# zju3dv/pats

Hardware: AMD Instinct MI355X
Metric: image-pairs/sec (coarse+fine OT) on 640x480 MegaDepth; OT iters/sec per pair (higher is better)
Workload: dtype f32 (contractions: fp32 operands split into fp16 hi + lo, three exact-product MFMA passes, fp32 accumulate)

## Files before the change

### include/pats_amd.h

```cpp
#ifndef PATS_AMD_H
#define PATS_AMD_H

#include <stddef.h>
#include <stdint.h>

#ifdef __cplusplus
extern "C" {
#endif

typedef void* pats_stream_t;

enum {
    PATS_OK = 0,
    PATS_ERR_INVALID = 1,
    PATS_ERR_UNSUPPORTED = 2,
    PATS_ERR_LAUNCH = 3,
    PATS_ERR_NO_DEVICE = 4
};

enum { PATS_SINKHORN_AUTO = 0, PATS_SINKHORN_LOG = 1, PATS_SINKHORN_KERNEL = 2 };

const char* pats_version(void);
#define PATS_ABI_VERSION 8
int pats_abi_version(void);
// ... 230 lines not shown
int pats_third_inputs_f32(const uint8_t* if_nomatching, const float* pts, int64_t B, float* mkpts0,
                          float* mkpts1, int64_t* b_ids, int64_t capacity, int64_t* count, void* workspace,
                          size_t workspace_bytes, pats_stream_t stream);

int pats_refine_scatter_f32(const uint8_t* if_nomatching, const float* pts, const float* mkpts1_f,
                            const float* label, int label_stride, int64_t B, int64_t P,
                            uint8_t* if_nomatching16, float* pts16, void* workspace,
                            size_t workspace_bytes, pats_stream_t stream);

size_t pats_get_result_workspace_bytes(int64_t cells0, int64_t rows1, int64_t cells1);
int pats_get_result_f32(int batch_size, const uint8_t* if_nomatching0, const uint8_t* if_nomatching1,
                        int64_t rows1, const float* average_point0, const float* average_point1,
                        const float* scale0, const float* scale1, int64_t scale1_cell_stride,
                        const int* patch_size0, const int* patch_size1, const uint8_t* left_choice0,
                        const uint8_t* left_choice1, float* matches_l, float* matches_r, int64_t capacity,
                        int64_t* count, void* workspace, size_t workspace_bytes, pats_stream_t stream);

int pats_get_result_chunks_f32(int Cmax, int64_t pairs, const uint8_t* masks, const uint8_t* if_nomatching16,
                               int64_t rows_cap, const float* pts_new, const float* pts16, const float* scales,
                               const int* patch_size0, const int* patch_size1, const uint8_t* left_choice0,
                               const uint8_t* left_choice1, float* matches_l, float* matches_r, int32_t* match_row,
                               int64_t capacity, int64_t* count, void* workspace, size_t workspace_bytes,
                               pats_stream_t stream);

size_t pats_matches_by_pair_workspace_bytes(int Cmax, int64_t pairs);
int pats_matches_by_pair_f32(const float* matches_l, const float* matches_r, const int32_t* match_row, const int64_t* M_dev,
                             const int32_t* row_cell, const int64_t* chunk_base, int Cmax, int64_t pairs, int N,
                             float* out_l, float* out_r, int64_t* pair_off, void* workspace, size_t workspace_bytes,
                             pats_stream_t stream);
int pats_matches_by_pair_summary_f32(const float* matches_l, const float* matches_r, const int32_t* match_row, const int64_t* M_dev,
                                     const int32_t* row_cell, const int64_t* chunk_base, int Cmax, int64_t pairs, int N,
                                     float* out_l, float* out_r, int64_t* pair_off, const int64_t* P_dev, const int32_t* status,
                                     void* workspace, size_t workspace_bytes, pats_stream_t stream);

typedef struct pats_pair_table {
    int64_t pairs;
    const int32_t* shape_host;
    const int64_t* cell_base_host;
    const int32_t* shape;
    const int64_t* cell_base;
    const int64_t* img_base;
} pats_pair_table_t;

int pats_chunk_rows_ragged(const pats_pair_table_t* tab, const uint8_t* if_nomatching1, int if_local, int Cmax, int64_t rows_cap,
                           int32_t* sum_cycle, int32_t* cycle_num, int64_t* second, int64_t* third, uint8_t* masks,
                           int64_t* chunk_base, int64_t* crop_base, int32_t* row_cell, int32_t* row_pair, uint8_t* row_forced,
                           int32_t* row_crop, int32_t* row_slot, int32_t* status, void* workspace, size_t workspace_bytes,
                           pats_stream_t stream);
int pats_compute_imgs_bounds_ragged_f32(const pats_pair_table_t* tab, const float* x_scale, const float* y_scale,
                                        const float* average_point, const uint8_t* if_nomatching, int64_t* bound5, int64_t* K_img,
                                        int64_t* K_total, float* x_scale_new, float* y_scale_new, float* average_new,
                                        pats_stream_t stream);
int pats_left_crops_ragged_f32(const pats_pair_table_t* tab, const float* left, const int64_t* bound5, int64_t K_cap,
                               const int64_t* K_dev, float* out, pats_stream_t stream);
int pats_tensor_resize_hwc_ragged_f32(const pats_pair_table_t* tab, const float* right, int margin, const int64_t* bound5,
                                      int64_t K_cap, const int64_t* K_dev, float* out, int32_t* status, pats_stream_t stream);

typedef enum { PATS_IMG_F32 = 0, PATS_IMG_F16 = 1, PATS_IMG_BF16 = 2, PATS_IMG_U8 = 3 } pats_img_dtype_t;
typedef enum { PATS_CROP_HWC = 0, PATS_CROP_CHW = 1 } pats_crop_layout_t;
typedef struct pats_crop_format {
    int32_t dtype;
    int32_t layout;
    int32_t normalize;
    float mean[3];
    float std[3];
} pats_crop_format_t;
// ... 309 lines not shown
```

### pats_amd/_lib.py

```python
import ctypes
import os

_HERE = os.path.dirname(os.path.abspath(__file__))
LIB_PATH = os.path.join(_HERE, "libpats_amd.so")
if os.environ.get("PATS_AMD_DIAG_LIB", "") not in ("", "0"):
    _sfx = os.environ["PATS_AMD_DIAG_LIB"]
    LIB_PATH = os.path.join(_HERE, "libpats_amd_diag%s.so" % ("" if _sfx == "1" else _sfx))

c_void_p, c_int, c_i64, c_f, c_size = (ctypes.c_void_p, ctypes.c_int, ctypes.c_int64, ctypes.c_float,
                                       ctypes.c_size_t)

ABI_VERSION = 8



class PairTable(ctypes.Structure):
    _fields_ = [("pairs", ctypes.c_int64), ("shape_host", c_void_p), ("cell_base_host", c_void_p), ("shape", c_void_p),
                ("cell_base", c_void_p), ("img_base", c_void_p)]


_TAB = ctypes.POINTER(PairTable)


class CropFormat(ctypes.Structure):
# ... 124 lines not shown
                                          c_i64, c_void_p, c_int, c_int, c_void_p, c_void_p, c_void_p] + [c_void_p] * 10 +
                                  [c_void_p, c_size, c_void_p]),
    "pats_get_result_chunks_f32": (c_int, [c_int, c_i64, c_void_p, c_void_p, c_i64, c_void_p, c_void_p, c_void_p,
                                           ctypes.POINTER(c_int), ctypes.POINTER(c_int), c_void_p, c_void_p, c_void_p,
                                           c_void_p, c_void_p, c_i64, c_void_p, c_void_p, c_size, c_void_p]),
    "pats_merge_workspace_bytes": (c_size, [c_i64, c_int, c_int, c_int]),
    "pats_merge_patches": (c_int, [c_int, c_i64, c_void_p, c_int, c_int, c_int, c_void_p, c_void_p, c_void_p,
                                   c_void_p, c_void_p, c_size, c_void_p]),
    "pats_compact_workspace_bytes": (c_size, [c_i64]),
    "pats_third_inputs_f32": (c_int, [c_void_p, c_void_p, c_i64, c_void_p, c_void_p, c_void_p, c_i64, c_void_p,
                                      c_void_p, c_size, c_void_p]),
    "pats_refine_scatter_f32": (c_int, [c_void_p, c_void_p, c_void_p, c_void_p, c_int, c_i64, c_i64, c_void_p,
                                        c_void_p, c_void_p, c_size, c_void_p]),
    "pats_attention_f32": (c_int, [c_void_p, c_void_p, c_void_p, c_i64, c_int, c_int, c_int, c_int, c_void_p, c_void_p,
                                   c_void_p]),
    "pats_attentional_propagation_workspace_bytes": (c_size, [c_i64, c_int, c_int, c_int]),
    "pats_attentional_propagation_f32": (c_int, [c_void_p, c_void_p, c_i64, c_int, c_int, c_int, c_int, c_void_p, c_int, c_f,
                                                 c_void_p, c_void_p, c_void_p, c_size, c_void_p]),
    "pats_propagation_packed_bytes": (c_size, [c_int, c_int]),
    "pats_propagation_pack_f32": (c_int, [c_void_p, c_int, c_int, c_void_p, c_size, c_void_p]),
    "pats_attentional_propagation_packed_f32": (c_int, [c_void_p, c_void_p, c_i64, c_int, c_int, c_int, c_int, c_void_p, c_void_p,
                                                        c_int, c_f, c_void_p, c_void_p, c_void_p, c_size, c_void_p]),
    "pats_attentional_gnn_packed_workspace_bytes": (c_size, [c_i64, c_int, c_int, c_int]),
    "pats_attentional_gnn_packed_f32": (c_int, [c_void_p, c_void_p, c_i64, c_void_p, c_i64, c_int, c_int, c_int, c_int, c_void_p, c_void_p,
                                                c_void_p, c_f, c_void_p, c_void_p, c_void_p, c_size, c_void_p]),
    "pats_attentional_propagation_packed_counted_f32": (c_int, [c_void_p, c_void_p, c_i64, c_void_p, c_i64, c_int, c_int, c_int, c_int,
                                                                c_void_p, c_void_p, c_int, c_f, c_void_p, c_void_p, c_void_p, c_size,
                                                                c_void_p]),
    "pats_matches_by_pair_workspace_bytes": (c_size, [c_int, c_i64]),
    "pats_matches_by_pair_f32": (c_int, [c_void_p, c_void_p, c_void_p, c_void_p, c_void_p, c_void_p, c_int, c_i64, c_int,
                                         c_void_p, c_void_p, c_void_p, c_void_p, c_size, c_void_p]),
    "pats_matches_by_pair_summary_f32": (c_int, [c_void_p, c_void_p, c_void_p, c_void_p, c_void_p, c_void_p, c_int, c_i64, c_int,
                                                 c_void_p, c_void_p, c_void_p, c_void_p, c_void_p, c_void_p, c_size, c_void_p]),
    "pats_chunk_rows_ragged": (c_int, [_TAB, c_void_p, c_int, c_int, c_i64] + [c_void_p] * 14 + [c_size, c_void_p]),
    "pats_compute_imgs_bounds_ragged_f32": (c_int, [_TAB] + [c_void_p] * 10 + [c_void_p]),
    "pats_left_crops_ragged_f32": (c_int, [_TAB, c_void_p, c_void_p, c_i64, c_void_p, c_void_p, c_void_p]),
    "pats_tensor_resize_hwc_ragged_f32": (c_int, [_TAB, c_void_p, c_int, c_void_p, c_i64, c_void_p, c_void_p, c_void_p, c_void_p]),
    "pats_left_crops_typed": (c_int, [_TAB, c_void_p, c_int, c_int, c_int, c_int, c_int, c_int, c_void_p, c_i64, c_void_p,
                                      _FMT, c_void_p, c_void_p]),
    "pats_tensor_resize_hwc_typed": (c_int, [_TAB, c_void_p, c_int, c_int, c_int, c_int, c_int, c_void_p, c_i64, c_void_p, _FMT,
                                             c_void_p, c_void_p, c_void_p]),
    "pats_tensor_resize_typed": (c_int, [c_void_p, c_int, c_int, c_int, c_int, c_int, c_void_p, c_i64, c_void_p, _FMT, c_void_p,
                                         c_void_p, c_void_p]),
    "pats_merge_ragged_workspace_bytes": (c_size, [c_i64]),
    "pats_merge_patches_ragged": (c_int, [_TAB, c_int, c_int, c_i64] + [c_void_p] * 8 + [c_int, c_void_p, c_void_p, c_size, c_void_p]),
    "pats_get_result_chunks_ragged_f32": (c_int, [_TAB, c_int, c_void_p, c_void_p, c_i64, c_void_p, c_void_p, c_void_p,
                                                  ctypes.POINTER(c_int), c_void_p, c_void_p, c_void_p, c_void_p, c_void_p, c_i64,
                                                  c_void_p, c_void_p, c_size, c_void_p]),
    "pats_matches_by_row_pair_summary_f32": (c_int, [c_void_p, c_void_p, c_void_p, c_void_p, c_void_p, c_void_p, c_int, c_i64,
                                                     c_void_p, c_void_p, c_void_p, c_void_p, c_void_p, c_void_p, c_size, c_void_p]),
    "pats_prepare_images_max_side": (c_i64, []),
    "pats_prepare_images_u8": (c_int, [c_void_p, c_void_p, c_i64, c_void_p, c_i64, c_void_p, c_i64, c_int, c_void_p]),
    "pats_third_level_typed_conf": (c_int, [c_void_p, c_void_p, c_int, c_i64, c_void_p, c_int, c_void_p, c_void_p, c_void_p, c_void_p,
                                            c_void_p, c_int, c_int, c_void_p, c_void_p, c_void_p, c_void_p, c_void_p, c_void_p,
                                            c_void_p]),
    "pats_compute_result_ws_conf_f32": (c_int, [c_void_p, c_int, c_i64, c_void_p, c_void_p, c_void_p, c_void_p,
                                                c_int, c_void_p, c_void_p, c_void_p, c_void_p, c_void_p, c_void_p,
                                                c_void_p, c_size, c_void_p]),
    "pats_refine_scatter_conf_f32": (c_int, [c_void_p, c_void_p, c_void_p, c_void_p, c_int, c_void_p, c_i64, c_i64, c_void_p,
                                             c_void_p, c_void_p, c_void_p, c_size, c_void_p]),
    "pats_get_result_chunks_conf_f32": (c_int, [c_int, c_i64, c_void_p, c_void_p, c_i64, c_void_p, c_void_p, c_void_p, c_void_p,
                                                ctypes.POINTER(c_int), ctypes.POINTER(c_int), c_void_p, c_void_p, c_void_p,
                                                c_void_p, c_void_p, c_void_p, c_i64, c_void_p, c_void_p, c_size, c_void_p]),
    "pats_get_result_chunks_ragged_conf_f32": (c_int, [_TAB, c_int, c_void_p, c_void_p, c_i64, c_void_p, c_void_p, c_void_p, c_void_p,
                                                       ctypes.POINTER(c_int), c_void_p, c_void_p, c_void_p, c_void_p, c_void_p,
                                                       c_void_p, c_i64, c_void_p, c_void_p, c_size, c_void_p]),
# ... 128 lines not shown
```

### pats_amd/batch.py

```python
import numpy as np
import torch

from . import ops


class Capacities:

    def __init__(self, pairs, h, w, if_local=True, p_cap_per_pair=None, rows_cap=None):
        self.pairs, self.h, self.w = int(pairs), int(h), int(w)
        self.N = self.h * self.w
        self.chunk_cap = 2 * self.w if if_local else 512
        self.Cmax = ops.max_chunks(self.h, self.w, self.chunk_cap)
        self.rows_cap = self.pairs * (self.N + (self.Cmax - 1) * self.w) if rows_cap is None else int(rows_cap)
        per_pair = int(1.25 * 16 * self.N) if p_cap_per_pair is None else int(p_cap_per_pair)
        self.P_cap = self.pairs * per_pair


class MixedCapacities:

    def __init__(self, shapes, if_local=True, p_cap_per_pair=None, rows_cap=None):
        self.shapes = [(int(h), int(w)) for h, w in shapes]
        self.if_local = bool(if_local)
        if not self.shapes:
            raise ValueError("MixedCapacities: no pairs")
# ... 163 lines not shown
    if events is not None:
        em = torch.cuda.Event(enable_timing=True)
        em.record()
        events.setdefault("fine_mid", []).append(em)
        ops.set_cost_ot_mid_event(em)
    live = rows.chunk_base[-1:]
    Z2, cflag2 = ops.cost_ot(f0, f1, 2, _one(f0.device), ns2, iters, bias_k=2.0 if if_outdoor else 3.0, return_flags=True,
                             count=live)
    if e is not None:
        e.record()
    trust2, pts2, _, _, ifn_L2, _ = ops.est_position_second(Z2, sx, sy, [96, 96], 8, col_nomatch=cflag2, count=live)
    merged = ops.merge_patches_batch(merge_new, rows, trust2, (H, W), ifn_L2)
    mk0, mk1, b_ids, P = ops.third_inputs(merged, pts2, capacity=cap.P_cap, sync=False)
    return {"co": co, "merged": merged, "pts2": pts2, "P": P, "mk0": mk0, "mk1": mk1, "b_ids": b_ids,
            "stages": {"Z2": Z2, "trust2": trust2, "pts2": pts2, "ifn_L2": ifn_L2, "sx": sx, "sy": sy, "f0": f0,
                       "f1": f1, "ns2": ns2, "mk0": mk0, "mk1": mk1, "b_ids": b_ids}}


def third_gather_stage(fs, nets, cap):
    third = nets.third(fs["co"]["rows"], fs["mk0"], fs["mk1"], fs["b_ids"], fs["P"])
    feat0, feat1, scale3 = third[:3]
    p_s, p_t = third[3:5] if len(third) > 3 else (_round4(fs["mk0"], False), _round4(fs["mk1"], True))
    fs.update(feat0=feat0, feat1=feat1, scale3=scale3, p_s=p_s, p_t=p_t)
    fs["stages"].update(feat0=feat0, feat1=feat1, scale3=scale3, p_s=p_s, p_t=p_t)
    return fs


def fine_stage(co, nets, cap, if_outdoor=True, merge_new=True, iters=100, events=None):
    return third_gather_stage(fine_solve_stage(co, nets, cap, if_outdoor, merge_new, iters, events), nets, cap)


def third_stage(fs, nets, cap, if_outdoor=True, iters=100, events=None, confidence=False):
    co, rows, P = fs["co"], fs["co"]["rows"], fs["P"]
    e = _timed(events, "third")
    level = ops.third_level(fs["feat0"], fs["feat1"], fs["scale3"], fs["p_s"], fs["p_t"], outdoor=if_outdoor, iters=iters, count=P,
                            return_confidence=bool(confidence))
    m0f, m1f, label, ifm = level[:4]
    if e is not None:
        e.record()
    scattered = ops.refine_scatter(fs["merged"], fs["pts2"], m1f, label, conf=level[4] if confidence else None)
    ifn16, pts16 = scattered[:2]
    result = ops.get_result_chunks(rows, ifn16, co["avn"], pts16, co["xsn"], conf16=scattered[2] if confidence else None)
    ml, mr, mrow, M = result[:4]
    stages = dict(fs["stages"], m0f=m0f, m1f=m1f, label=label, ifm=ifm, pts16=pts16)
    out = {"matches_l": ml, "matches_r": mr, "match_row": mrow}
    if confidence:
        stages.update(conf=level[4], conf16=scattered[2])
        out["match_conf"] = result[4]
    out.update(M=M, P=P, status=rows.status, rows=rows, if_nomatching16=ifn16, merged=fs["merged"], K_img=co["K_img"],
               crops=(co["new_left"], co["new_right"]), coarse=co, stages=stages)
    return out


def fine_third_stage(co, nets, cap, if_outdoor=True, merge_new=True, iters=100, events=None, confidence=False):
    fs = fine_stage(co, nets, cap, if_outdoor, merge_new, iters, events)
    return third_stage(fs, nets, cap, if_outdoor, iters, events, confidence)


def forward_pairs(lefts, rights, nets, cap, if_outdoor=True, merge_new=True, iters=100, events=None, crop_format=None,
                  confidence=False):
    co = coarse_stage(lefts, rights, nets, cap, iters, fine_inputs=False, crop_format=crop_format)
    return fine_third_stage(co, nets, cap, if_outdoor, merge_new, iters, events, confidence)


def coarse_stage_mixed(pack, nets, cap, iters=100, if_local=True, crop_format=None):
    ifn1, xs, ys, pts = [], [], [], []
    for lo, hi, h, w, lefts, rights in pack.groups:
        _, p_, x_, y_, f_, _ = _coarse_tail(lefts, rights, nets, iters, 32 * h, 32 * w)
        ifn1.append(f_.reshape(-1))
        xs.append(x_.reshape(-1))
        ys.append(y_.reshape(-1))
        pts.append(p_.reshape(-1))
    one = len(pack.groups) == 1
    ifn1 = ifn1[0] if one else torch.cat(ifn1)
    xs, ys, pts = (xs[0], ys[0], pts[0]) if one else (torch.cat(xs), torch.cat(ys), torch.cat(pts))
    rows = ops.chunk_rows_ragged(ifn1, pack.table, if_local, Cmax=cap.Cmax, rows_cap=cap.rows_cap)
    new_left, new_right, xsn, ysn, avn, bound5, K_img, K_tot = ops.Compute_imgs_ragged(xs, ys, pts, ifn1, pack.left, pack.right,
                                                                                       pack.table, crop_format=crop_format)
    return {"rows": rows, "new_left": new_left, "new_right": new_right, "xsn": xsn, "avn": avn, "K_img": K_img, "ifn1": ifn1,
            "H": None, "W": None}


def forward_pairs_mixed(pack, nets, cap, if_outdoor=True, merge_new=True, iters=100, events=None, crop_format=None,
                        confidence=False):
    if cap.pairs != pack.table.pairs or sorted(cap.shapes) != sorted(pack.shapes):
        raise ValueError("forward_pairs_mixed: the capacities were made for other shapes than the pack holds")
    co = coarse_stage_mixed(pack, nets, cap, iters, cap.if_local, crop_format=crop_format)
    out = fine_third_stage(co, nets, cap, if_outdoor, merge_new, iters, events, confidence)
    out["caller_of"] = pack.caller_of
    return out


def group_by_pair(out, cap, buffers=None, confidence=False):
    if confidence and "match_conf" not in out:
        raise ValueError("group_by_pair: confidence=True needs a result made with confidence=True")
    got = ops.matches_by_pair(out["rows"], out["matches_l"], out["matches_r"], out["match_row"], out["M"], out=buffers, P=out["P"],
                              match_conf=out.get("match_conf"))
    out["by_pair"], out["summary"] = got[:3] + got[4:], got[3]
    return out["by_pair"]


def _overflow_check(o, cap):
    M, P, status = o[cap.pairs + 1:cap.pairs + 4]
    if status & 1:
        raise RuntimeError("pats_amd.batch: a pair needed more than Cmax = %d chunks" % cap.Cmax)
    if status & 2:
        raise RuntimeError("pats_amd.batch: the row table overflowed rows_cap = %d" % cap.rows_cap)
    if P > cap.P_cap:
        raise RuntimeError("pats_amd.batch: %d third-level problems exceed P_cap = %d" % (P, cap.P_cap))


def _read_topk_summary(out, cap):
    if "topk_summary" in out:
        o = out["topk_summary"].cpu().tolist()
        return o[:cap.pairs + 4], o[cap.pairs + 4:]
    return out["summary"].cpu().tolist(), out["topk"][4].cpu().tolist()


def _caller_order(out, cap, per_slot):
    if "caller_of" not in out:
        return per_slot
    per_caller = [None] * cap.pairs
    for s_, i in enumerate(out["caller_of"]):
        per_caller[i] = per_slot[s_]
    return per_caller


def _caller_of_dev(out, dev):
# ... 83 lines not shown
    g, most = grid(int(cell)), ops.topk_spread_max_cells()
    if g[0] * g[1] > most:
        fits = next(c for c in range(int(cell) + 1, max(H, W) + 1) if grid(c)[0] * grid(c)[1] <= most)
        raise ValueError("topk_spread_by_pair: cell = %d makes %d x %d cells on %d x %d pixels, more than max_cells = %d; the "
                         "smallest cell that fits is %d" % (cell, g[0], g[1], H, W, most, fits))
    return g


def topk_spread_by_pair(out, cap, K, cell, min_conf=None, side="left"):
    grid = _spread_grid(cap, cell)
    ml, mr, mc, top_count = _topk_lists("topk_spread_by_pair", out, cap)
    dest = None
    if top_count is not None:
        dest = _topk_dest(cap, K, ml.device, top_count) + (torch.empty((cap.pairs,), dtype=torch.int64, device=ml.device),)
    got = ops.topk_spread_by_pair(ml, mr, mc, out["summary"], K, int(cell), grid, side=side, min_conf=min_conf, out=dest, pairs=cap.pairs)
    out["topk"], out["topk_spread"] = got[:5], (got[5], int(cell), grid, side)
    return out["topk"]


def split_topk_by_pair(out, cap):
    if "topk" not in out:
        raise ValueError("split_topk_by_pair: run topk_by_pair first")
    tl, tr, tc, ti, _ = out["topk"]
    o, counts = _read_topk_summary(out, cap)
    _overflow_check(o, cap)
    per_slot = [(tl[p, :counts[p]], tr[p, :counts[p]], tc[p, :counts[p]], ti[p, :counts[p]]) for p in range(cap.pairs)]
    return _caller_order(out, cap, per_slot)


def _sample_by_pair(fn, generate, out, cap, H, seed, norm, on, progressive, samples):
    _check_on(fn, out, on)
    if progressive is None:
        progressive = on == "topk"
    dev = out["matches_l"].device
    seed = ((int(seed) + (1 << 63)) % (1 << 64)) - (1 << 63)
    mixed = "caller_of" in out
    if out.get("pair_seed", (None,))[0] != seed:
        ids = _caller_of_dev(out, dev) if mixed else torch.arange(cap.pairs, dtype=torch.int64, device=dev)
        out["pair_seed"] = (seed, ids + seed)
    pair_seed = out["pair_seed"][1]
    if mixed and norm is not None:
        norm = norm.index_select(0, _caller_of_dev(out, dev))
    ml, mr, _, seg = _lists_on(out, cap, on)
    hyp = generate(ml, mr, H, pair_seed, norm=norm, progressive=progressive, return_samples=samples, **seg)
    if mixed:
        back = _slot_of_dev(out, cap, dev)
        hyp = tuple(t.index_select(0, back) for t in hyp) if samples else hyp.index_select(0, back)
    return hyp


def hypothesize_by_pair(out, cap, H, seed=0, norm=None, on="topk", progressive=None, samples=False):
    hyp = _sample_by_pair("hypothesize_by_pair", ops.epipolar_hypotheses_by_pair, out, cap, H, seed, norm, on, progressive, samples)
    out["hypotheses"] = hyp
    return hyp


def hypothesize5_by_pair(out, cap, H, seed=0, norm=None, on="topk", progressive=None, samples=False):
    hyp = _sample_by_pair("hypothesize5_by_pair", ops.epipolar_hypotheses5_by_pair, out, cap, H, seed, norm, on, progressive, samples)
    flat = (hyp[0] if samples else hyp).flatten(1, 2)
    hyp = (flat, hyp[1]) if samples else flat
    out["hypotheses5"] = hyp
    return hyp


def hypothesize7_by_pair(out, cap, H, seed=0, norm=None, on="topk", progressive=None, samples=False):
    hyp = _sample_by_pair("hypothesize7_by_pair", ops.epipolar_hypotheses7_by_pair, out, cap, H, seed, norm, on, progressive, samples)
    out["hypotheses7"] = hyp
# ... 414 lines not shown
```

### pats_amd/build.py

```python
import os
import shutil
import subprocess
import sys

HERE = os.path.dirname(os.path.abspath(__file__))
CSRC = os.path.join(HERE, "csrc")
LIB = os.path.join(HERE, "libpats_amd.so")
LIB_DIAG = os.path.join(HERE, "libpats_amd_diag.so")
DIAG_SOURCES = None
SOURCES = ["host.cpp", "sinkhorn.hip", "sinkhorn_stream.hip", "sinkhorn_blk.hip", "sinkhorn_blk2w.hip", "cost.hip", "post.hip", "expand.hip", "resize.hip", "third.hip", "third_fused.hip", "third_fused3.hip", "gather.hip", "merge.hip", "attention.hip", "attention145.hip", "gnn.hip", "gnn_fused.hip", "gnn_fine.hip", "conv_pk.hip",
           "fused.hip", "scale_head.hip", "batch.hip", "topk.hip", "topk_spread.hip", "epipolar.hip", "hypotheses.hip", "hypotheses5.hip", "hypotheses7.hip", "pose.hip", "pose_h.hip", "triangulate.hip", "pose_error.hip", "homography.hip", "fundamental.hip", "adaptive.hip", "polish.hip", "prepare.hip", "absolute.hip", "chunk_walk.cpp"]
DIAG_SOURCES = {src: ["-DPATS_DIAG=1"] for src in SOURCES}
FLAGS = ["--offload-arch=gfx950", "-O3", "-std=c++17", "-fPIC", "-fno-fast-math", "-ffp-contract=off",
         "-Wall", "-Wno-unused-function", "-x", "hip"]
EXTRA_FLAGS = {"third_fused.hip": ["-fno-slp-vectorize"], "third_fused3.hip": ["-fno-slp-vectorize"],
               "cost.hip": ["-fno-slp-vectorize"], "gnn.hip": ["-fno-slp-vectorize"]}


def hipcc():
    exe = shutil.which("hipcc") or "/opt/rocm/bin/hipcc"
    if not os.path.exists(exe):
        raise RuntimeError("hipcc not found - libpats_amd.so cannot be built")
    return exe


def compile_tu(spath, obj, extra=(), verbose=False):
    cmd = [hipcc()] + FLAGS[:-2] + list(extra) + FLAGS[-2:] + ["-c", spath, "-o", obj]
    if verbose:
        print(" ".join(cmd))
    p = subprocess.run(cmd, stdout=subprocess.PIPE, stderr=subprocess.STDOUT)
    if p.returncode != 0:
        sys.stderr.write(p.stdout.decode())
        raise RuntimeError("hipcc failed on %s" % os.path.basename(spath))
    if verbose and p.stdout:
        print(p.stdout.decode())


def compile_many(jobs, verbose=False):
    from concurrent.futures import ThreadPoolExecutor
    with ThreadPoolExecutor(max_workers=min(8, max(1, len(jobs)))) as ex:
        futs = [ex.submit(compile_tu, s, o, e, verbose) for s, o, e in jobs]
        return [f.result() for f in futs]

# ... 91 lines not shown
```

### pats_amd/csrc/third_device.hpp

```cpp
#pragma once
#include "common.hpp"

namespace pats {

struct ComputeResultOut {
    float* mk0;
    float* mk1;
    float* wl_raw;
    float* label;
    uint8_t* ifm;
    int* count;
};

struct Fused65Args {
    const float* d0;
    const float* d1;
    int D;
    int64_t P;
    const float* ns;
    const float* one;
    int iters, linear;
    const float* scale_x;
    const float* scale_y;
    const int64_t* p_s;
// ... 4 lines not shown
    unsigned long long* fallbacks;
    int scan;
    const int64_t* P_dev;
    int fingerprint;
    int lds_poison_on;
    unsigned lds_poison;
    int reverse_blocks;
    int dtype;
};
__device__ __forceinline__ int64_t live_problems(const Fused65Args& g) {
    if (!g.P_dev) return g.P;
    const int64_t n = *g.P_dev;
    return n < g.P ? n : g.P;
}
constexpr uint8_t THIRD_REDO = 0xEE;
int launch_third_fused(const Fused65Args& g, hipStream_t st, float* conf = nullptr);

constexpr int SST = 36;
constexpr float GUARD = 1073741824.0f;
__device__ __forceinline__ bool sc_ok(float x) { return x <= GUARD && x > 0.f; }
__device__ __forceinline__ float uni(float x) { return __builtin_bit_cast(float, __builtin_amdgcn_readfirstlane(__builtin_bit_cast(int, x))); }

template <unsigned FRONT>
__device__ __forceinline__ void dephase_first_front(int stagger) {
    if (stagger > 0 && blockIdx.x < FRONT) {
        const unsigned slots = (blockIdx.x * 2654435761u) >> 29;
        for (unsigned q = 0; q < slots * (unsigned)stagger; ++q) __builtin_amdgcn_s_sleep(127);
    }
}

template <class Solve>
__device__ __forceinline__ void third_redo_walk(const Fused65Args& g, int lane, Solve&& solve) {
    const int64_t W = gridDim.x, live = live_problems(g);
    for (int64_t first = blockIdx.x; first < live; first += 64 * W) {
        const int64_t cand = first + (int64_t)lane * W;
        const bool redo = cand < live && g.cr.ifm[cand * 16] == THIRD_REDO;
        unsigned long long todo = __ballot(redo);
        while (todo) {
            const int k = __ffsll((long long)todo) - 1;
            todo &= todo - 1;
            wg_barrier();
            solve(first + (int64_t)k * W);
        }
    }
}
inline unsigned third_walk_grid(int64_t P) { return (unsigned)(P < 1 ? 1 : P < 6144 ? P : 6144); }

__device__ __forceinline__ float row16_sum(float v) {
    v += dpp_f<DPP_QUAD_XOR1>(v);
    v += dpp_f<DPP_QUAD_XOR2>(v);
    v += dpp_f<DPP_ROW_HALF_MIRROR>(v);
    v += dpp_f<DPP_ROW_MIRROR>(v);
    return v;
}
template <int CTRL>
__device__ __forceinline__ void argmax_step(float& v, int& i) {
    const float ov = dpp_f<CTRL>(v);
    const int oi = dpp_i<CTRL>(i);
    if (ov > v || (ov == v && oi < i)) { v = ov; i = oi; }
}
__device__ __forceinline__ void row16_argmax(float& v, int& i) {
    argmax_step<DPP_QUAD_XOR1>(v, i);
    argmax_step<DPP_QUAD_XOR2>(v, i);
    argmax_step<DPP_ROW_HALF_MIRROR>(v, i);
    argmax_step<DPP_ROW_MIRROR>(v, i);
}
// ... 101 lines not shown
```

### pats_amd/ops.py

```python
import collections
import ctypes

import numpy as np
import torch

from . import _lib

_L = _lib.lib
_check = _lib.check
_L()


_raw_stream = getattr(torch._C, "_cuda_getCurrentRawStream", None)


def _stream():
    if _raw_stream is not None:
        return ctypes.c_void_p(_raw_stream(torch.cuda.current_device()))
    return ctypes.c_void_p(torch.cuda.current_stream().cuda_stream)


def _dev(t, name, dtype=torch.float32):
    if not isinstance(t, torch.Tensor):
        raise TypeError("%s must be a torch.Tensor" % name)
# ... 1235 lines not shown
                      ("pats_get_result_chunks_ragged_f32", "pats_get_result_chunks_ragged_conf_f32"))
_MATCHES_BY_PAIR = (("pats_matches_by_pair_summary_f32", "pats_matches_by_pair_summary_conf_f32"),
                    ("pats_matches_by_row_pair_summary_f32", "pats_matches_by_row_pair_summary_conf_f32"))


def matches_by_pair(rows, matches_l, matches_r, match_row, M, out=None, P=None, match_conf=None):
    dev = matches_l.device
    n_off = rows.pairs + 1 + (3 if P is not None else 0)
    if out is None:
        out = (torch.empty_like(matches_l), torch.empty_like(matches_r), torch.empty((n_off,), dtype=torch.int64, device=dev))
    ol, orr, off = out[:3]
    if off.numel() != n_off or not off.is_contiguous():
        raise RuntimeError("matches_by_pair: pair_off must be a contiguous int64 tensor of %d entries" % n_off)
    nws = _L().pats_matches_by_pair_workspace_bytes(rows.Cmax, rows.pairs)
    ws = _workspace(nws, dev)
    mc_arg, oc_arg, res = (), (), ((ol, orr, off) if P is None else (ol, orr, off[:rows.pairs + 1], off))
    if match_conf is not None:
        mc = _dev(match_conf, "match_conf").reshape(-1)
        oc = out[3] if len(out) > 3 else torch.empty_like(mc)
        if mc.numel() != matches_l.shape[0] or oc.numel() != mc.numel() or oc.dtype != torch.float32 or not oc.is_contiguous():
            raise RuntimeError("matches_by_pair: match_conf and its destination must be contiguous float32 [cap] tensors")
        mc_arg, oc_arg, res = (_ptr(mc),), (_ptr(oc),), res + (oc,)
    pair_args = (_ptr(rows.row_pair),) if rows.table is not None else (_ptr(rows.row_cell),)
    grid_arg = () if rows.table is not None else (rows.h * rows.w,)
    if P is None and match_conf is None and rows.table is None:
        entry, tail = "pats_matches_by_pair_f32", ()
    else:
        entry = _MATCHES_BY_PAIR[rows.table is not None][match_conf is not None]
        tail = (_ptr(_dev(P, "P", torch.int64)), _ptr(rows.status)) if P is not None else (None, None)
    _check(getattr(_L(), entry)(_ptr(matches_l), _ptr(matches_r), *mc_arg, _ptr(match_row), _ptr(M), *pair_args, _ptr(rows.chunk_base),
                                rows.Cmax, rows.pairs, *grid_arg, _ptr(ol), _ptr(orr), *oc_arg, _ptr(off), *tail, _ptr(ws), nws,
                                _stream()), "matches_by_pair")
    return res


def _bp_layout(fn, named, types=()):
    types = dict(types)
    for t, name in named:
        if not isinstance(t, torch.Tensor):
            continue
        if not t.is_contiguous():
            raise RuntimeError("%s: %s must be contiguous" % (fn, name))
        want = types.get(name, torch.float32)
        if t.dtype != want:
            raise RuntimeError("%s: %s must be %s, got %s" % (fn, name, str(want).replace("torch.", ""), t.dtype))


def _bp_one_form(fn, pair_off, stride, counts):
    if (pair_off is None) == (counts is None) or (stride is None) != (counts is None):
        raise RuntimeError("%s: give either pair_off, or stride and counts" % fn)


_Family = collections.namedtuple("_Family", "first width same_shape lists model models letter moments cost")
_EPI = _Family("matches_l", 2, True, "matches_l / matches_r must be [cap,2]", (3, 3), "[pairs,H,3,3]", "H", True, False)
_ABS = _Family("points", 3, False, "points must be [cap,3] and matches_r [cap,2]", (3, 4), "[pairs,M,3,4]", "M", False, True)


def _bp_flat(t, width):
    shape = t.shape
    if len(shape) < 2 or shape[-1] != width:
        return None
    return t if len(shape) == 2 else t.reshape(-1, width)


def _bp_vector(t, name, dtype=torch.float32):
    t = _dev(t, name, dtype)
# ... 1358 lines not shown
```

Before: 1934.

## Fuse refine scatter, result chunking and pair grouping into a single tail pass

Adds a four-kernel result-tail path (cell prefix, per-row counts, segment offsets, scatter write) that produces per-pair grouped matches directly from the merged mask and third-level labels. It skips the separate refine_scatter, get_result_chunks and matches_by_pair steps, which are now computed lazily only when a caller asks for those outputs. The redo walk in the third-stage kernel also exits early when no problem is flagged for redo. In exchange it adds a single-block offsets kernel and duplicated match-coordinate math that must stay consistent with the old chain.

```diff
diff --git a/include/pats_amd.h b/include/pats_amd.h
--- a/include/pats_amd.h
+++ b/include/pats_amd.h
@@ -286,6 +286,13 @@
                                      const int32_t* row_cell, const int64_t* chunk_base, int Cmax, int64_t pairs, int N,
                                      float* out_l, float* out_r, int64_t* pair_off, const int64_t* P_dev, const int32_t* status,
                                      void* workspace, size_t workspace_bytes, pats_stream_t stream);
+
+size_t pats_result_tail_workspace_bytes(int Cmax, int64_t pairs, int64_t rows_cap);
+int pats_result_tail_by_pair_f32(const uint8_t* merged, const float* mkpts1_f, const float* label, int label_stride, int64_t P_rows,
+                                 const int32_t* row_cell, const int64_t* chunk_base, int Cmax, int64_t pairs, int h, int w,
+                                 int64_t rows_cap, const float* pts_new, const float* scales, const int64_t* P_dev,
+                                 const int32_t* status, float* out_l, float* out_r, int64_t* pair_off, int32_t* match_row,
+                                 int64_t* M_dev, int64_t capacity, void* workspace, size_t workspace_bytes, pats_stream_t stream);
 
 typedef struct pats_pair_table {
     int64_t pairs;
diff --git a/pats_amd/_lib.py b/pats_amd/_lib.py
--- a/pats_amd/_lib.py
+++ b/pats_amd/_lib.py
@@ -180,6 +180,10 @@
                                          c_void_p, c_void_p, c_void_p, c_void_p, c_size, c_void_p]),
     "pats_matches_by_pair_summary_f32": (c_int, [c_void_p, c_void_p, c_void_p, c_void_p, c_void_p, c_void_p, c_int, c_i64, c_int,
                                                  c_void_p, c_void_p, c_void_p, c_void_p, c_void_p, c_void_p, c_size, c_void_p]),
+    "pats_result_tail_workspace_bytes": (c_size, [c_int, c_i64, c_i64]),
+    "pats_result_tail_by_pair_f32": (c_int, [c_void_p, c_void_p, c_void_p, c_int, c_i64, c_void_p, c_void_p, c_int, c_i64, c_int, c_int,
+                                             c_i64, c_void_p, c_void_p, c_void_p, c_void_p, c_void_p, c_void_p, c_void_p, c_void_p,
+                                             c_void_p, c_i64, c_void_p, c_size, c_void_p]),
     "pats_chunk_rows_ragged": (c_int, [_TAB, c_void_p, c_int, c_int, c_i64] + [c_void_p] * 14 + [c_size, c_void_p]),
     "pats_compute_imgs_bounds_ragged_f32": (c_int, [_TAB] + [c_void_p] * 10 + [c_void_p]),
     "pats_left_crops_ragged_f32": (c_int, [_TAB, c_void_p, c_void_p, c_i64, c_void_p, c_void_p, c_void_p]),
diff --git a/pats_amd/batch.py b/pats_amd/batch.py
--- a/pats_amd/batch.py
+++ b/pats_amd/batch.py
@@ -219,6 +219,8 @@
 
 def third_stage(fs, nets, cap, if_outdoor=True, iters=100, events=None, confidence=False):
     co, rows, P = fs["co"], fs["co"]["rows"], fs["P"]
+    if not confidence and rows.table is None:
+        return _third_stage_fused(fs, nets, cap, if_outdoor, iters, events)
     e = _timed(events, "third")
     level = ops.third_level(fs["feat0"], fs["feat1"], fs["scale3"], fs["p_s"], fs["p_t"], outdoor=if_outdoor, iters=iters, count=P,
                             return_confidence=bool(confidence))
@@ -239,6 +241,47 @@
     return out
 
 
+class _ChainEntries:
+
+    def __init__(self, rows, merged, pts2, m1f, label, avn, xsn):
+        self.args, self.made = (rows, merged, pts2, m1f, label, avn, xsn), None
+
+    def get(self):
+        if self.made is None:
+            rows, merged, pts2, m1f, label, avn, xsn = self.args
+            ifn16, pts16 = ops.refine_scatter(merged, pts2, m1f, label)
+            ml, mr = ops.get_result_chunks(rows, ifn16, avn, pts16, xsn)[:2]
+            self.made = {"matches_l": ml, "matches_r": mr, "if_nomatching16": ifn16, "pts16": pts16}
+        return self.made
+
+
+class _OnDemand(dict):
+    source, on_demand = None, ()
+
+    def __missing__(self, key):
+        if key not in self.on_demand:
+            raise KeyError(key)
+        self[key] = self.source.get()[key]
+        return dict.__getitem__(self, key)
+
+
+def _third_stage_fused(fs, nets, cap, if_outdoor, iters, events):
+    co, rows, P = fs["co"], fs["co"]["rows"], fs["P"]
+    e = _timed(events, "third")
+    m0f, m1f, label, ifm = ops.third_level(fs["feat0"], fs["feat1"], fs["scale3"], fs["p_s"], fs["p_t"], outdoor=if_outdoor, iters=iters,
+                                           count=P)[:4]
+    if e is not None:
+        e.record()
+    bl, br, pair_off, summary, mrow, M = ops.result_tail_by_pair(rows, fs["merged"], m1f, label, co["avn"], co["xsn"], P)
+    stages = _OnDemand(fs["stages"], m0f=m0f, m1f=m1f, label=label, ifm=ifm)
+    out = _OnDemand(match_row=mrow, M=M, P=P, status=rows.status, rows=rows, merged=fs["merged"], K_img=co["K_img"],
+                    crops=(co["new_left"], co["new_right"]), coarse=co, stages=stages, tail=(bl, br, pair_off, summary))
+
+    out.source = stages.source = _ChainEntries(rows, fs["merged"], fs["pts2"], m1f, label, co["avn"], co["xsn"])
+    out.on_demand, stages.on_demand = ("matches_l", "matches_r", "if_nomatching16"), ("pts16",)
+    return out
+
+
 def fine_third_stage(co, nets, cap, if_outdoor=True, merge_new=True, iters=100, events=None, confidence=False):
     fs = fine_stage(co, nets, cap, if_outdoor, merge_new, iters, events)
     return third_stage(fs, nets, cap, if_outdoor, iters, events, confidence)
@@ -281,6 +324,14 @@
 def group_by_pair(out, cap, buffers=None, confidence=False):
     if confidence and "match_conf" not in out:
         raise ValueError("group_by_pair: confidence=True needs a result made with confidence=True")
+    if "tail" in out:
+        got = out["tail"]
+        if buffers is not None:
+            st, co = out["stages"], out["coarse"]
+            got = ops.result_tail_by_pair(out["rows"], out["merged"], st["m1f"], st["label"], co["avn"], co["xsn"], out["P"],
+                                          out=tuple(buffers[:3]) + (out["match_row"],))[:4]
+        out["by_pair"], out["summary"] = got[:3], got[3]
+        return out["by_pair"]
     got = ops.matches_by_pair(out["rows"], out["matches_l"], out["matches_r"], out["match_row"], out["M"], out=buffers, P=out["P"],
                               match_conf=out.get("match_conf"))
     out["by_pair"], out["summary"] = got[:3] + got[4:], got[3]
@@ -430,7 +481,7 @@
     _check_on(fn, out, on)
     if progressive is None:
         progressive = on == "topk"
-    dev = out["matches_l"].device
+    dev = (out["tail"][0] if "tail" in out else out["matches_l"]).device
     seed = ((int(seed) + (1 << 63)) % (1 << 64)) - (1 << 63)
     mixed = "caller_of" in out
     if out.get("pair_seed", (None,))[0] != seed:
diff --git a/pats_amd/build.py b/pats_amd/build.py
--- a/pats_amd/build.py
+++ b/pats_amd/build.py
@@ -8,7 +8,7 @@
 LIB = os.path.join(HERE, "libpats_amd.so")
 LIB_DIAG = os.path.join(HERE, "libpats_amd_diag.so")
 DIAG_SOURCES = None
-SOURCES = ["host.cpp", "sinkhorn.hip", "sinkhorn_stream.hip", "sinkhorn_blk.hip", "sinkhorn_blk2w.hip", "cost.hip", "post.hip", "expand.hip", "resize.hip", "third.hip", "third_fused.hip", "third_fused3.hip", "gather.hip", "merge.hip", "attention.hip", "attention145.hip", "gnn.hip", "gnn_fused.hip", "gnn_fine.hip", "conv_pk.hip",
+SOURCES = ["host.cpp", "sinkhorn.hip", "sinkhorn_stream.hip", "sinkhorn_blk.hip", "sinkhorn_blk2w.hip", "cost.hip", "post.hip", "expand.hip", "resize.hip", "third.hip", "third_fused.hip", "third_fused3.hip", "gather.hip", "merge.hip", "result_tail.hip", "attention.hip", "attention145.hip", "gnn.hip", "gnn_fused.hip", "gnn_fine.hip", "conv_pk.hip",
            "fused.hip", "scale_head.hip", "batch.hip", "topk.hip", "topk_spread.hip", "epipolar.hip", "hypotheses.hip", "hypotheses5.hip", "hypotheses7.hip", "pose.hip", "pose_h.hip", "triangulate.hip", "pose_error.hip", "homography.hip", "fundamental.hip", "adaptive.hip", "polish.hip", "prepare.hip", "absolute.hip", "chunk_walk.cpp"]
 DIAG_SOURCES = {src: ["-DPATS_DIAG=1"] for src in SOURCES}
 FLAGS = ["--offload-arch=gfx950", "-O3", "-std=c++17", "-fPIC", "-fno-fast-math", "-ffp-contract=off",
diff --git a/pats_amd/csrc/result_tail.hip b/pats_amd/csrc/result_tail.hip
--- /dev/null
+++ b/pats_amd/csrc/result_tail.hip
@@ -0,0 +1,316 @@
+#include "common.hpp"
+
+namespace pats {
+
+constexpr int TAIL_TILE = 256;
+constexpr int TAIL_SEG_LDS = 4096;
+constexpr int TAIL_ROWS = 4;
+
+struct TailArgs {
+    const uint8_t* merged;
+    const float* mkpts1; const float* label; int label_stride; int64_t P_rows;
+    const int32_t* row_cell; const int64_t* chunk_base; int Cmax; int64_t pairs; int h, w;
+    const float* ap0; const float* sc0;
+    const int64_t* P_dev; const int32_t* status;
+    int64_t rows_cap, capacity;
+    float* out_l; float* out_r; int64_t* pair_off; int32_t* match_row; int64_t* M_dev;
+    int32_t* cell_pfx; int32_t* tile_tot; int32_t* row_cnt; int32_t* row_base;
+    int32_t* row_key;
+    int64_t* seg_lo; int64_t* seg_hi; int64_t* seg_dst;
+    int32_t* seg_first; int32_t* seg_last;
+};
+
+__device__ __forceinline__ int tail_incl_scan(int v, int lane) {
+#pragma unroll
+    for (int d = 1; d < 64; d <<= 1) {
+        const int o = __shfl_up(v, d);
+        if (lane >= d) v += o;
+    }
+    return v;
+}
+
+__device__ __forceinline__ int zero_bytes(uint32_t x) {
+    uint32_t y = x | (x >> 4);
+    y |= y >> 2;
+    y |= y >> 1;
+    return 4 - __popc(y & 0x01010101u);
+}
+
+__device__ __forceinline__ bool tail_live(const TailArgs& g, int64_t k) {
+    const int32_t e = g.row_cell[k];
+    return e >= 0 && e < g.pairs * ((int64_t)g.h * g.w);
+}
+__device__ __forceinline__ int64_t tail_key(const TailArgs& g, int64_t k) {
+    int c = 0;
+    for (int q = 1; q < g.Cmax; ++q) c += (k >= g.chunk_base[q]) ? 1 : 0;
+    return (int64_t)c * g.pairs + g.row_cell[k] / (g.h * g.w);
+}
+
+__global__ void __launch_bounds__(256)
+tail_cells_kernel(TailArgs g) {
+    __shared__ int wsum[4];
+    const int t = threadIdx.x, lane = t & 63, wave = t >> 6;
+    const int64_t k = (int64_t)blockIdx.x * TAIL_TILE + t;
+    for (int64_t s = k; s < 2 * (int64_t)g.Cmax * g.pairs; s += (int64_t)gridDim.x * TAIL_TILE) g.seg_first[s] = -1;
+    int c = 0;
+    if (k < g.rows_cap) {
+        const uint4* row = reinterpret_cast<const uint4*>(g.merged + k * 144);
+#pragma unroll
+        for (int q = 0; q < 9; ++q) {
+            const uint4 v = row[q];
+            c += zero_bytes(v.x) + zero_bytes(v.y) + zero_bytes(v.z) + zero_bytes(v.w);
+        }
+    }
+    const int incl = tail_incl_scan(c, lane);
+    if (lane == 63) wsum[wave] = incl;
+    wg_barrier();
+    int base = 0;
+    for (int w2 = 0; w2 < wave; ++w2) base += wsum[w2];
+    if (k < g.rows_cap) {
+        g.cell_pfx[k] = base + incl - c;
+        g.row_key[k] = tail_live(g, k) ? (int32_t)tail_key(g, k) : -1;
+    }
+    if (t == 255 && (int64_t)blockIdx.x * TAIL_TILE < g.rows_cap) g.tile_tot[blockIdx.x] = base + incl;
+}
+
+__device__ __forceinline__ void tail_row_cells(const TailArgs& g, int64_t k, int lane, int32_t* cellP) {
+    int part = 0;
+    for (int64_t b = lane; b < k / TAIL_TILE; b += 64) part += g.tile_tot[b];
+#pragma unroll
+    for (int off = 32; off; off >>= 1) part += __shfl_xor(part, off);
+    int64_t P = (int64_t)part + g.cell_pfx[k];
+#pragma unroll
+    for (int m = 0; m < 3; ++m) {
+        const int cell = 64 * m + lane;
+        const bool kept = cell < 144 && g.merged[k * 144 + cell] == 0;
+        const uint64_t bal = __builtin_amdgcn_ballot_w64(kept);
+        if (cell < 144) {
+            const int64_t mine = P + __popcll(bal & ((1ull << lane) - 1ull));
+            cellP[cell] = kept && mine < g.P_rows ? (int32_t)mine : -1;
+        }
+        P += __popcll(bal);
+    }
+    wave_lds_sync();
+}
+constexpr int TAIL_HALF = 18;
+__device__ __forceinline__ void tail_keep_half(const TailArgs& g, int64_t k, int lane, const int32_t* cellP, int i0, uint64_t (&words)[TAIL_HALF]) {
+    const float* const idle = reinterpret_cast<const float*>(g.row_cell + k);
+    float lab[TAIL_HALF];
+    uint32_t has = 0;
+#pragma unroll
+    for (int u = 0; u < TAIL_HALF; ++u) {
+        const int j = 64 * (i0 + u) + lane, yy = j / 48, xx = j - yy * 48;
+        const int32_t p = cellP[(yy >> 2) * 12 + (xx >> 2)];
+        lab[u] = *(p >= 0 ? g.label + ((int64_t)p * 16 + (yy & 3) * 4 + (xx & 3)) * g.label_stride : idle);
+        has |= (uint32_t)(p >= 0) << u;
+    }
+#pragma unroll
+    for (int u = 0; u < TAIL_HALF; ++u) words[u] = __builtin_amdgcn_ballot_w64(((has >> u) & 1u) != 0 && !(lab[u] < -9.9f));
+}
+
+__global__ void __launch_bounds__(64 * TAIL_ROWS) __attribute__((amdgpu_waves_per_eu(4)))
+tail_count_kernel(TailArgs g) {
+    __shared__ int32_t cellP[TAIL_ROWS][144];
+    const int lane = threadIdx.x & 63, wave = threadIdx.x >> 6;
+    const int64_t k = (int64_t)blockIdx.x * TAIL_ROWS + __builtin_amdgcn_readfirstlane(wave);
+    if (k >= g.rows_cap) return;
+    const int32_t key = g.row_key[k], before = k > 0 ? g.row_key[k - 1] : -1, behind = k + 1 < g.rows_cap ? g.row_key[k + 1] : -1;
+    if (key < 0) {
+        if (lane == 0) g.row_cnt[k] = 0;
+        return;
+    }
+    {
+        const bool first = before != key, last = behind != key;
+        if (first && lane == 0) g.seg_first[key] = (int32_t)k;
+        if (last && lane == 0) g.seg_last[key] = (int32_t)k;
+    }
+    tail_row_cells(g, k, lane, cellP[wave]);
+    int c = 0;
+#pragma unroll
+    for (int i0 = 0; i0 < 36; i0 += TAIL_HALF) {
+        uint64_t words[TAIL_HALF];
+        tail_keep_half(g, k, lane, cellP[wave], i0, words);
+#pragma unroll
+        for (int u = 0; u < TAIL_HALF; ++u) c += __popcll(words[u]);
+        __builtin_amdgcn_sched_barrier(0);
+    }
+    if (lane == 0) g.row_cnt[k] = c;
+}
+
+__global__ void __launch_bounds__(1024)
+tail_offsets_kernel(TailArgs g) {
+    __shared__ int wsum[16];
+    __shared__ int psum[16];
+    __shared__ int64_t carry;
+    __shared__ int seg_n[TAIL_SEG_LDS];
+    const int t = threadIdx.x, lane = t & 63, wave = t >> 6;
+    const int32_t* __restrict__ cnt = g.row_cnt;
+    int32_t* __restrict__ rb = g.row_base;
+    const int64_t chunk = ((g.rows_cap + 1023) / 1024) * 64, k0 = wave * chunk, k1 = k0 + chunk < g.rows_cap ? k0 + chunk : g.rows_cap;
+    int c = 0;
+    for (int64_t k = k0 + lane; k < k1; k += 64) c += cnt[k];
+#pragma unroll
+    for (int off = 32; off; off >>= 1) c += __shfl_xor(c, off);
+    if (lane == 0) wsum[wave] = c;
+    if (t == 0) carry = 0;
+    wg_barrier();
+    int run = 0, all = 0;
+    for (int w2 = 0; w2 < 16; ++w2) { if (w2 < wave) run += wsum[w2]; all += wsum[w2]; }
+    for (int64_t kb = k0; kb < k1; kb += 64) {
+        const int64_t k = kb + lane;
+        const int v = k < k1 ? cnt[k] : 0, incl = tail_incl_scan(v, lane);
+        if (k < k1) rb[k] = run + incl - v;
+        run += __shfl(incl, 63);
+    }
+    wg_barrier_global();
+    const int64_t P = g.pairs, nseg = g.Cmax * P;
+    for (int64_t s = t; s < nseg; s += 1024) {
+        const int32_t first = g.seg_first[s], last = g.seg_last[s];
+        const int64_t lo = first >= 0 ? rb[first] : 0, hi = last >= 0 ? (int64_t)rb[last] + cnt[last] : 0;
+        g.seg_lo[s] = lo;
+        g.seg_hi[s] = hi;
+        if (s < TAIL_SEG_LDS) seg_n[s] = (int)(hi - lo);
+    }
+    const auto run_size = [&](int64_t s) -> int64_t { return s < TAIL_SEG_LDS ? seg_n[s] : g.seg_hi[s] - g.seg_lo[s]; };
+    wg_barrier_global();
+    for (int64_t p0 = 0; p0 < P; p0 += 1024) {
+        const int64_t p = p0 + t;
+        int tt = 0;
+        if (p < P)
+            for (int q = 0; q < g.Cmax; ++q) tt += (int)run_size(q * P + p);
+        const int incl2 = tail_incl_scan(tt, lane);
+        if (lane == 63) psum[wave] = incl2;
+        wg_barrier();
+        int64_t off = carry;
+        int round = 0;
+        for (int w2 = 0; w2 < 16; ++w2) { if (w2 < wave) off += psum[w2]; round += psum[w2]; }
+        off += incl2 - tt;
+        if (p < P) {
+            g.pair_off[p] = off;
+            for (int q = 0; q < g.Cmax; ++q) { g.seg_dst[q * P + p] = off; off += run_size(q * P + p); }
+        }
+        wg_barrier();
+        if (t == 0) carry += round;
+    }
+    wg_barrier();
+    if (t == 0) {
+        g.pair_off[P] = carry;
+        g.pair_off[P + 1] = all;
+        g.pair_off[P + 2] = g.P_dev ? *g.P_dev : 0;
+        g.pair_off[P + 3] = (int64_t)*g.status;
+        *g.M_dev = all;
+    }
+}
+
+__global__ void __launch_bounds__(64 * TAIL_ROWS) __attribute__((amdgpu_waves_per_eu(4)))
+tail_write_kernel(TailArgs g) {
+    __shared__ int32_t cellP[TAIL_ROWS][144];
+    const int lane = threadIdx.x & 63, wave = threadIdx.x >> 6;
+    const int64_t k = (int64_t)blockIdx.x * TAIL_ROWS + __builtin_amdgcn_readfirstlane(wave);
+    if (k >= g.rows_cap) return;
+    const int32_t key = g.row_key[k];
+    if (key < 0 || g.row_cnt[k] == 0) return;
+    const int64_t e = g.row_cell[k];
+    const unsigned i0 = (unsigned)(e % (g.h * g.w)), w0 = (unsigned)g.w;
+    const int64_t mbase = g.row_base[k], dbase = g.seg_dst[key] + (mbase - g.seg_lo[key]);
+    const float z0 = 32.0f, z1 = 2.0f;
+    const float sc_l = g.sc0[e * 2 + 1], sc_r = g.sc0[e * 2];
+    float l0[2], r0[2];
+#pragma unroll
+    for (int d = 0; d < 2; ++d) {
+        const float pos0 = (float)((d == 0 ? i0 / w0 : i0 % w0) * 32u);
+        float dl0 = pos0 + 0.5f * z0;
+        dl0 = dl0 - (1.5f * sc_l) * z0;
+        const float a0 = g.ap0[e * 2 + (1 - d)] / 32.0f;
+        const float dr0 = (a0 - 1.5f * sc_r) * z0;
+        l0[d] = 0.0f + dl0;
+        r0[d] = 0.0f + dr0;
+    }
+    tail_row_cells(g, k, lane, cellP[wave]);
+    const float2* const idle = reinterpret_cast<const float2*>(g.sc0 + e * 2);
+    int run = 0;
+#pragma unroll
+    for (int ib = 0; ib < 36; ib += TAIL_HALF) {
+        uint64_t words[TAIL_HALF];
+        tail_keep_half(g, k, lane, cellP[wave], ib, words);
+        float2 pts[TAIL_HALF];
+#pragma unroll
+        for (int u = 0; u < TAIL_HALF; ++u) {
+            const int j = 64 * (ib + u) + lane, yy = j / 48, xx = j - yy * 48;
+            const int64_t s = (int64_t)cellP[wave][(yy >> 2) * 12 + (xx >> 2)] * 16 + (yy & 3) * 4 + (xx & 3);
+            pts[u] = *((words[u] >> lane) & 1ull ? reinterpret_cast<const float2*>(g.mkpts1) + s : idle);
+        }
+#pragma unroll
+        for (int u = 0; u < TAIL_HALF; ++u) {
+            const int r = run + __popcll(words[u] & ((1ull << lane) - 1ull));
+            run += __popcll(words[u]);
+            const int64_t M = mbase + r, dst = dbase + r;
+            if (!((words[u] >> lane) & 1ull) || M >= g.capacity || dst < 0 || dst >= g.capacity) continue;
+            const int j = 64 * (ib + u) + lane, yy = j / 48, xx = j - yy * 48;
+            const float2 pt = pts[u];
+            float2 ml, mr;
+#pragma unroll
+            for (int d = 0; d < 2; ++d) {
+                const float a1 = (d == 0 ? pt.y : pt.x) / 2.0f;
+                const float pos1 = (float)((unsigned)(d == 0 ? yy : xx) * 2u);
+                float dl1 = pos1 + 0.5f * z1;
+                dl1 = dl1 * sc_l;
+                const float dr1 = (a1 * z1) * sc_r;
+                (d == 0 ? ml.x : ml.y) = l0[d] + dl1;
+                (d == 0 ? mr.x : mr.y) = r0[d] + dr1;
+            }
+            reinterpret_cast<float2*>(g.out_l)[dst] = ml;
+            reinterpret_cast<float2*>(g.out_r)[dst] = mr;
+            g.match_row[M] = (int32_t)k;
+        }
+        __builtin_amdgcn_sched_barrier(0);
+    }
+}
+
+}
+
+using namespace pats;
+
+static size_t tail_rows4(int64_t rows_cap) { return (size_t)((rows_cap + 3) & ~3ll); }
+static int64_t tail_tiles(int64_t rows_cap) { return (rows_cap + TAIL_TILE - 1) / TAIL_TILE; }
+
+extern "C" size_t pats_result_tail_workspace_bytes(int Cmax, int64_t pairs, int64_t rows_cap) {
+    if (Cmax < 1 || pairs < 1 || rows_cap < 0) return 0;
+    const size_t nseg = (size_t)Cmax * pairs;
+    return nseg * 3 * sizeof(int64_t) + (4 * tail_rows4(rows_cap) + tail_rows4(tail_tiles(rows_cap)) + 2 * nseg) * sizeof(int32_t) + 64;
+}
+
+extern "C" int pats_result_tail_by_pair_f32(const uint8_t* merged, const float* mkpts1_f, const float* label, int label_stride,
+                                            int64_t P_rows, const int32_t* row_cell, const int64_t* chunk_base, int Cmax, int64_t pairs,
+                                            int h, int w, int64_t rows_cap, const float* pts_new, const float* scales,
+                                            const int64_t* P_dev, const int32_t* status, float* out_l, float* out_r, int64_t* pair_off,
+                                            int32_t* match_row, int64_t* M_dev, int64_t capacity, void* workspace,
+                                            size_t workspace_bytes, pats_stream_t stream) {
+    PATS_REQUIRE(Cmax >= 1 && pairs >= 1 && h >= 1 && w >= 1 && rows_cap >= 0 && P_rows >= 0 && capacity >= 0 && label_stride >= 1,
+                 "result_tail_by_pair: bad shape");
+    PATS_REQUIRE(pairs * (int64_t)h * w < (1ll << 31) && rows_cap * 2304 < (1ll << 31) && P_rows < (1ll << 27) &&
+                 Cmax * pairs < (1ll << 28), "result_tail_by_pair: batch too large");
+    PATS_REQUIRE(row_cell && chunk_base && pts_new && scales && status && pair_off && M_dev && (rows_cap == 0 || merged) &&
+                 (P_rows == 0 || (mkpts1_f && label)) && (capacity == 0 || (out_l && out_r && match_row)),
+                 "result_tail_by_pair: null pointer");
+    PATS_REQUIRE_ALIGNED("result_tail_by_pair", merged, 16);
+    PATS_REQUIRE_ALIGNED("result_tail_by_pair", mkpts1_f, 8);
+    PATS_REQUIRE_ALIGNED("result_tail_by_pair", out_l, 8);
+    PATS_REQUIRE_ALIGNED("result_tail_by_pair", out_r, 8);
+    PATS_REQUIRE(workspace && (uintptr_t)workspace % 8 == 0 && workspace_bytes >= pats_result_tail_workspace_bytes(Cmax, pairs, rows_cap),
+                 "result_tail_by_pair: workspace too small or misaligned");
+    hipStream_t st = as_stream(stream);
+    const int64_t nseg = (int64_t)Cmax * pairs, tiles = tail_tiles(rows_cap), groups = (rows_cap + TAIL_ROWS - 1) / TAIL_ROWS;
+    int64_t* seg = reinterpret_cast<int64_t*>(workspace);
+    int32_t* per_row = reinterpret_cast<int32_t*>(seg + 3 * nseg);
+    const size_t r4 = tail_rows4(rows_cap);
+    int32_t* ends = per_row + 4 * r4 + tail_rows4(tiles);
+    TailArgs g{merged, mkpts1_f, label, label_stride, P_rows, row_cell, chunk_base, Cmax, pairs, h, w, pts_new, scales, P_dev, status,
+               rows_cap, capacity, out_l, out_r, pair_off, match_row, M_dev,
+               per_row, per_row + 4 * r4, per_row + r4, per_row + 2 * r4, per_row + 3 * r4, seg, seg + nseg, seg + 2 * nseg, ends, ends + nseg};
+    hipLaunchKernelGGL(tail_cells_kernel, dim3((unsigned)(tiles > 0 ? tiles : 1)), dim3(TAIL_TILE), 0, st, g);
+    if (rows_cap > 0) hipLaunchKernelGGL(tail_count_kernel, dim3((unsigned)groups), dim3(64 * TAIL_ROWS), 0, st, g);
+    hipLaunchKernelGGL(tail_offsets_kernel, dim3(1), dim3(1024), 0, st, g);
+    if (rows_cap > 0 && capacity > 0) hipLaunchKernelGGL(tail_write_kernel, dim3((unsigned)groups), dim3(64 * TAIL_ROWS), 0, st, g);
+    return check_launch("result_tail_by_pair kernels");
+}
diff --git a/pats_amd/csrc/third_device.hpp b/pats_amd/csrc/third_device.hpp
--- a/pats_amd/csrc/third_device.hpp
+++ b/pats_amd/csrc/third_device.hpp
@@ -60,6 +60,12 @@
 template <class Solve>
 __device__ __forceinline__ void third_redo_walk(const Fused65Args& g, int lane, Solve&& solve) {
     const int64_t W = gridDim.x, live = live_problems(g);
+    bool any = false;
+    for (int64_t first = blockIdx.x; first < live; first += 64 * W) {
+        const int64_t cand = first + (int64_t)lane * W;
+        any |= __ballot(cand < live && g.cr.ifm[cand * 16] == THIRD_REDO) != 0ull;
+    }
+    if (!any) return;
     for (int64_t first = blockIdx.x; first < live; first += 64 * W) {
         const int64_t cand = first + (int64_t)lane * W;
         const bool redo = cand < live && g.cr.ifm[cand * 16] == THIRD_REDO;
diff --git a/pats_amd/ops.py b/pats_amd/ops.py
--- a/pats_amd/ops.py
+++ b/pats_amd/ops.py
@@ -1291,6 +1291,48 @@
                                 rows.Cmax, rows.pairs, *grid_arg, _ptr(ol), _ptr(orr), *oc_arg, _ptr(off), *tail, _ptr(ws), nws,
                                 _stream()), "matches_by_pair")
     return res
+
+
+def result_tail_by_pair(rows, if_nomatching, mkpts1_f, label, pts_new, scales, P=None, out=None, capacity=None):
+    if rows.table is not None:
+        raise RuntimeError("result_tail_by_pair: a ragged table goes through refine_scatter / get_result_chunks / matches_by_pair")
+    f = _as_flags(if_nomatching, "if_nomatching")
+    if f.numel() != rows.rows_cap * 144:
+        raise RuntimeError("result_tail_by_pair: if_nomatching must be [rows_cap,144]")
+    mk = _dev(mkpts1_f, "mkpts1_f").reshape(-1, 16, 2)
+    P_rows = mk.shape[0]
+    lb = _dev(label, "label")
+    stride = 2 if lb.dim() == 2 else 1
+    if lb.numel() != P_rows * 16 * stride:
+        raise RuntimeError("result_tail_by_pair: label must be [P*16,2] or [P*16]")
+    a0, s0 = _dev(pts_new, "pts_new"), _dev(scales, "scales")
+    cells = rows.pairs * rows.h * rows.w
+    if a0.numel() != cells * 2 or s0.numel() != cells * 2:
+        raise RuntimeError("result_tail_by_pair: pts_new / scales must be [pairs,N,2]")
+    dev = a0.device
+    cap = rows.rows_cap * 2304 if capacity is None else int(capacity)
+    n_off = rows.pairs + 4
+    if out is None:
+        out = (torch.empty((cap, 2), dtype=torch.float32, device=dev), torch.empty((cap, 2), dtype=torch.float32, device=dev),
+               torch.empty((n_off,), dtype=torch.int64, device=dev))
+    ol, orr, off = out[:3]
+    if off.numel() != n_off or off.dtype != torch.int64 or not off.is_contiguous():
+        raise RuntimeError("result_tail_by_pair: summary must be a contiguous int64 tensor of %d entries" % n_off)
+    for t, name in ((ol, "out_l"), (orr, "out_r")):
+        if t.dtype != torch.float32 or not t.is_contiguous() or t.numel() < cap * 2:
+            raise RuntimeError("result_tail_by_pair: %s must be a contiguous float32 [cap,2] tensor" % name)
+    mrow = out[3] if len(out) > 3 else torch.empty((cap,), dtype=torch.int32, device=dev)
+    if mrow.dtype != torch.int32 or not mrow.is_contiguous() or mrow.numel() < cap:
+        raise RuntimeError("result_tail_by_pair: match_row must be a contiguous int32 [cap] tensor")
+    cnt = torch.empty((1,), dtype=torch.int64, device=dev)
+    nws = _L().pats_result_tail_workspace_bytes(rows.Cmax, rows.pairs, rows.rows_cap)
+    ws = _workspace(nws, dev)
+    _check(_L().pats_result_tail_by_pair_f32(_ptr(f), _ptr(mk), _ptr(lb), stride, P_rows, _ptr(rows.row_cell), _ptr(rows.chunk_base),
+                                             rows.Cmax, rows.pairs, rows.h, rows.w, rows.rows_cap, _ptr(a0), _ptr(s0),
+                                             _ptr(_dev(P, "P", torch.int64)) if P is not None else None, _ptr(rows.status), _ptr(ol),
+                                             _ptr(orr), _ptr(off), _ptr(mrow), _ptr(cnt), cap, _ptr(ws), nws, _stream()),
+           "result_tail_by_pair")
+    return ol, orr, off[:rows.pairs + 1], off, mrow, cnt
 
 
 def _bp_layout(fn, named, types=()):
```

New measurement: 1946, median of 2. No clear change (+0.6%).
